# petim0/fly_bProject

Hardware: AMD Instinct MI355X
Metric: env-steps/sec (PPO rollout + update), 8192 envs per GPU (higher is better)
Workload: dtype f32 (optimizer step: fp16x2 operand split; rollout policy + critic: bf16x3 operand split; fp32 accumulate)

## Files before the change

### fly_bproject_amd/_lib.py

```python
import ctypes as C
import os

from .params import FlyParams

_HERE = os.path.dirname(os.path.abspath(__file__))
LIB_PATH = os.environ.get("FLYHIP_LIB") or os.path.join(_HERE, "libflyhip.so")
_lib = None


class FlyHipError(RuntimeError):
    pass


class FlyBuffers(C.Structure):
    _fields_ = [(n, C.c_void_p) for n in ("root", "dof_state", "targets", "contact", "pot", "prev_pot",
                                          "obs", "reward", "reset", "progress", "ep_return", "ep_length",
                                          "done_return", "done_length", "done_count")]


class FlyRenderConfig(C.Structure):
    _fields_ = [("width", C.c_int32), ("height", C.c_int32), ("fov_y_deg", C.c_float), ("cam_offset", C.c_float * 3),
                ("look_z", C.c_float)]


# ... 32 lines not shown
    "ppo_rollout_step": [_P, _P, _P, _P, _P, _P, _P, _I, _F, _F, _P, _P, _P, _P, _P, _P],
    "ppo_rollout_all": [_P, _P, _P, _P, _P, _P, _P, _F, _F, _P, _P, _P, _P, _I, _P, _P, _P, _P, _P],
    "ppo_rollout_bookkeeping": [_P, _L, _L, _P, _P, _F, _P, _I, _F, _F, _P, _P],
    "mlp_forward": [_P, _P, _P, _L, _P, _P, _P, _P, _P, _P, _P, _P],
    "mlp_forward_sample": [_P, _P, _P, _L, _P, _P, _I, _F, _F, _P, _P, _P, _P, _P, _P],
    "mlp_grad_workspace_floats": [],
    "mlp_backward_dx": [_P] * 10 + [_L, _F, _F, _P, _P, _P, _P, _P, _P, _P],
    "mlp_forward_backward": [_P] * 4 + [_L] + [_P] * 9 + [_F, _F] + [_P] * 6 + [_I, _P, _P, _P, _I, _P],
    "mlp_grad_w": [_P] * 8 + [_L, _P, _P, _P, _P, _P, _P, _I, _P],
    "mlp_fused_workspace_floats": [],
    "mlp_fused_grad": [_P] * 3 + [_P, _L] + [_P] * 5 + [_F, _F] + [_P] * 6 + [C.POINTER(_P), _P],
    "mlp_fused_h2_workspace_floats": [],
    "mlp_fused_grad_h2": [_P] * 5 + [_I, _P, _L] + [_P] * 5 + [_F, _F] + [_P] * 6 + [C.POINTER(_P), _P],
    "mlp_h2_rescale": [_P] * 7,
    "mlp_adam_step": [_P] * 10 + [_F, _F, _F, _F, _F, _F, _P, _I, _P, _P, _P, _P, _P, _P] + [_P] * 3 + [_I, _P],
    "dqn_eps_greedy": [_P, _P, _P, _F, _I, _P, _L, _P],
    "dqn_huber_td": [_P, _P, _P, _P, _P, _F, _I, _L, _P, _P, _P],
    "dqn_forward": [_P, _P, _P, _L, _P, _P],
    "dqn_act": [_P, _P, _P, _L, _P, _P, _F, _P, _P, _P],
    "dqn_td_step": [_P] * 10 + [_L, _F, _F] + [_P] * 7,
    "dqn_grad_workspace_floats": [],
    "dqn_grad_w": [_P] * 6 + [_L, _P, _P, _I, _P],
    "dqn_fused_workspace_floats": [],
    "dqn_fused_image_halves": [_L],
    "dqn_fused_update": [_P] * 6 + [_I, _L, _F, _F, _P, _P, _P, _P, _I, _P],
    "dqn_fused_h2_workspace_floats": [],
    "dqn_fused_h2_image_halves": [_L],
    "dqn_fused_update_h2": [_P] * 10 + [_I, _L, _F, _F, _P, _P, _P, _P, _I, _I, _P],
    "dqn_adam_soft_update": [_P] * 12 + [_F, _F, _F, _F, _F, _P, _P, _P, _P, _P, _P, _P],
    "dp_p2p_alloc": [_L, C.POINTER(_P)],
# ... 48 lines not shown
```

### fly_bproject_amd/csrc/flyhip_abi.hip

```cpp
#include <hip/hip_runtime.h>
#include <string.h>
#include <stdint.h>
#include <stdio.h>
#include <stdarg.h>
#include <new>
#include "flyhip.h"
#include "obs_norm.h"
#include "domain_rand.h"
#include <math.h>

extern "C" hipError_t flyhip_launch_env(int phases, const FlyConfig* dcfg, int n, const float* actions,
                                        const FlyBuffers* b, void* stream, int dr);
extern "C" hipError_t flyhip_launch_sample_logprob(const float* mu, const float* var, const float* eps,
                                                   float* act_out, float* logp_out, int64_t n, void* stream);
extern "C" hipError_t flyhip_launch_td_gae(const float* reward, const float* v, const float* v_next,
                                           const float* done, float gamma, float lambda, int64_t T, int64_t N,
                                           float* target_out, float* adv_out, int mode, void* stream);

extern "C" hipError_t flyhip_launch_mlp_forward(const float* P, const float* PF, const float* x, int64_t n, float* mu_out,
                                                float* v_out, float* out_save, float* h1_save, float* h2_save,
                                                float* h3_save, const uint16_t* PB, void* stream);

extern "C" hipError_t flyhip_launch_mlp_backward_dx(const float* PT, const float* out_saved, const float* h1,
                                                    const float* h2, const float* h3, const float* action,
// ... 27 lines not shown
                                                   int64_t n, const float* action, const float* old_logp, const float* adv,
                                                   const float* target, const float* var, float inv_batch, float clip,
                                                   float* workspace, float* grad_out, const float* norm_mask, float* norm_ws,
                                                   int* norm_step, float* loss_part, float* const* dump, void* stream);
extern "C" hipError_t flyhip_launch_mlp_grad_w(const float* x, const float* h1, const float* h2, const float* h3,
                                               const float* dz1, const float* dz2, const float* dz3, const float* dz4,
                                               int64_t n, float* workspace, float* grad_out, const float* norm_mask,
                                               float* norm_ws, int* norm_step, const int* err, int gemm_b3, void* stream);
extern "C" hipError_t flyhip_launch_mlp_adam(float* P, float* PF, float* PT, const int* idx_f, const int* idx_t,
                                             const float* G, const float* mask, float* m,
                                             float* v, int* step, float lr, float beta1, float beta2, float eps,
                                             float max_norm, float grad_scale, float* norm_ws, int norm_ready,
                                             uint16_t* PB, uint16_t* PTB, const int* idx_fb, const int* idx_tb,
                                             int* step_out, const int* grad_invalid, uint16_t* PH, uint16_t* PTH,
                                             float* h2_scales, int h2_period, void* stream);
extern "C" hipError_t flyhip_launch_mlp_h2_rescale(const float* P, const int* idx_fb, const int* idx_tb, uint16_t* PH, uint16_t* PTH,
                                                   float* h2_scales, void* stream);
extern "C" int64_t flyhip_mlp_fused_h2_workspace_floats(void);
extern "C" hipError_t flyhip_launch_mlp_fused_grad_h2(const float* P, const uint16_t* PH, const uint16_t* PTH, float* fsc, int* ovf,
                                                      int freeze, const float* x, int64_t n, const float* action,
                                                      const float* old_logp, const float* adv, const float* target, const float* var,
                                                      float inv_batch, float clip, float* workspace, float* grad_out,
                                                      const float* norm_mask, float* norm_ws, int* norm_step, float* loss_part,
                                                      float* const* dump, void* stream);

extern "C" hipError_t flyhip_launch_bookkeeping(const float* reward, int64_t n, float* score_acc, float score_scale,
                                                float* action_var, int nvar, float var_decay, float var_min,
                                                void* stream);

extern "C" hipError_t flyhip_launch_dqn_eps_greedy(const float* q, const float* coin_u, const float* rand_u, float epsilon,
// ... 527 lines not shown
{
    if (params_b3 && (!params_t_b3 || !idx_b3 || !idx_t_b3))
        return fail(FLY_E_ARG, "mlp_adam_step: params_b3 needs params_t_b3, idx_b3 and idx_t_b3");
    if (params_h2 && (!params_t_h2 || !h2_scales || !params_b3))
        return fail(FLY_E_ARG, "mlp_adam_step: params_h2 needs params_t_h2, h2_scales and the bf16x3 planes with their index maps");
    if (!params || !params_frag || !params_t_frag || !idx_frag || !idx_t_frag || !grad || !mask || !exp_avg ||
        !exp_avg_sq || !step || !norm_ws)
        return fail(FLY_E_ARG, "mlp_adam_step: null pointer");
    hipError_t e = flyhip_launch_mlp_adam(params, params_frag, params_t_frag, idx_frag, idx_t_frag, grad, mask, exp_avg, exp_avg_sq, step, lr, beta1, beta2,
                                          eps, max_norm, grad_scale, norm_ws, norm_ready, params_b3, params_t_b3, idx_b3, idx_t_b3,
                                          step_out, grad_invalid, params_h2, params_t_h2, h2_scales, h2_period, stream);
    if (e != hipSuccess) return hip_fail(e, "mlp_adam_step launch");
    return FLY_OK;
}

int dqn_eps_greedy(const float* q, const float* coin_u, const float* rand_u, float epsilon, int32_t A,
                   float* act_out, int64_t n, void* stream)
{
    if (!q || !coin_u || !rand_u || !act_out) return fail(FLY_E_ARG, "dqn_eps_greedy: null pointer");
    if (n <= 0 || A < 2) return fail(FLY_E_ARG, "dqn_eps_greedy: need n > 0 and A >= 2");
    hipError_t e = flyhip_launch_dqn_eps_greedy(q, coin_u, rand_u, epsilon, A, act_out, n, stream);
    if (e != hipSuccess) return hip_fail(e, "dqn_eps_greedy launch");
    return FLY_OK;
}

int dqn_huber_td(const float* q_table, const float* act, const float* reward, const float* q_next,
                 const float* done, float discount, int32_t A, int64_t B, float* dq, float* loss_part,
                 void* stream)
{
    if (!q_table || !act || !reward || !q_next || !done || !dq || !loss_part)
// ... 190 lines not shown
```

### fly_bproject_amd/csrc/mlp_adam.inc

```
constexpr int ADAM_THREADS = 1024;
constexpr int ADAM_WAVES = ADAM_THREADS / 64;
constexpr int ADAM_BLOCKS = (MLP_PACKED_FLOATS + ADAM_THREADS - 1) / ADAM_THREADS;

constexpr int H2_SINCE = 40;
constexpr int H2_WMAX = 64;
constexpr int H2_WMAX_SLOTS = (MLP_PACKED_FLOATS + 63) / 64;
constexpr int H2_TABLE_FLOATS = H2_WMAX + 2 * H2_WMAX_SLOTS;
__device__ __forceinline__ int h2_group_layer(int w)
{
    const int o = 64 * w;
    return o < MLP_OFF_B1 ? 0 : o < MLP_OFF_W2 ? -1 : o < MLP_OFF_B2 ? 1 : o < MLP_OFF_W3 ? -1 : o < MLP_OFF_B3 ? 2 : o < MLP_OFF_W4 ? -1
         : o < MLP_OFF_B4 ? 3 : -1;
}
__device__ __forceinline__ float h2_wave_max(float x)
{
    x = fmaxf(x, __builtin_bit_cast(float, __builtin_amdgcn_update_dpp(0, __builtin_bit_cast(int, x), 0xB1, 0xF, 0xF, true)));
    x = fmaxf(x, __builtin_bit_cast(float, __builtin_amdgcn_update_dpp(0, __builtin_bit_cast(int, x), 0x4E, 0xF, 0xF, true)));
    x = fmaxf(x, __builtin_bit_cast(float, __builtin_amdgcn_update_dpp(0, __builtin_bit_cast(int, x), 0x141, 0xF, 0xF, true)));
    x = fmaxf(x, __builtin_bit_cast(float, __builtin_amdgcn_update_dpp(0, __builtin_bit_cast(int, x), 0x140, 0xF, 0xF, true)));
    const int b = __builtin_bit_cast(int, x);
    return fmaxf(fmaxf(__builtin_bit_cast(float, __builtin_amdgcn_readlane(b, 0)), __builtin_bit_cast(float, __builtin_amdgcn_readlane(b, 16))),
                 fmaxf(__builtin_bit_cast(float, __builtin_amdgcn_readlane(b, 32)), __builtin_bit_cast(float, __builtin_amdgcn_readlane(b, 48))));
}
static_assert(MLP_OFF_B1 % 64 == 0 && MLP_OFF_W2 % 64 == 0 && MLP_OFF_B2 % 64 == 0 && MLP_OFF_W3 % 64 == 0 && MLP_OFF_B3 % 64 == 0 &&
// ... 153 lines not shown
            const _Float16 h1 = (_Float16)(ps - (float)h0);
            const u16 a = __builtin_bit_cast(u16, h0), b = __builtin_bit_cast(u16, h1);
            const int hf = (kf / 1536) * 1024 + kf % 1536;
            PH[hf] = a; PH[hf + 512] = b;
            if (kt >= 0) { const int ht = (kt / 1536) * 1024 + kt % 1536; PTH[ht] = a; PTH[ht + 512] = b; }
        }
    }
    if (PH) {
        const int w = i >> 6;
        float mw = 0.0f;
        if (h2_group_layer(w) >= 0) mw = h2_wave_max(fabsf(p));
        if ((tid & 63) == 0 && w < H2_WMAX_SLOTS) fsc[H2_WMAX + par * H2_WMAX_SLOTS + w] = mw;
    }
}

constexpr int H2_RESCALE_THREADS = 1024;
__global__ __launch_bounds__(H2_RESCALE_THREADS) void mlp_h2_rescale_kernel(const float* __restrict__ P, const int* __restrict__ idx_fb,
                                                                            const int* __restrict__ idx_tb, u16* __restrict__ PH,
                                                                            u16* __restrict__ PTH, float* __restrict__ fsc)
{
    __shared__ unsigned s_max[4];
    __shared__ float s_scale[4];
    const int tid = threadIdx.x;
    if (tid < 4) s_max[tid] = 0u;
    __syncthreads();
    float mine[4] = {0.0f, 0.0f, 0.0f, 0.0f};
    for (int i = tid; i < MLP_PACKED_FLOATS; i += H2_RESCALE_THREADS)
        if (idx_fb[i] >= 0) {
            const int layer = i < MLP_OFF_W2 ? 0 : i < MLP_OFF_W3 ? 1 : i < MLP_OFF_W4 ? 2 : 3;
            const float a = fabsf(P[i]);
// ... 42 lines not shown
```

### fly_bproject_amd/csrc/mlp_mfma.hip

```cpp
#include <hip/hip_runtime.h>
#include <stdint.h>
#include <type_traits>
#include <cstdio>
#include <cstdlib>
#include "flyhip.h"
#include "mlp_layout.h"
#include "obs_norm.h"
#include "domain_rand.h"

namespace {

#include "mlp_gemm.inc"
#include "fs_stamp.inc"
#include "mlp_forward.inc"
#include "mlp_backward.inc"
#include "mlp_grad_w.inc"
#include "mlp_fused_step.inc"
#include "mlp_adam.inc"
#include "fly_body.inc"

constexpr int RS_LDS_FLOATS = FWD_LDS_FLOATS > ENVS_PER_BLOCK * FLY_NUM_OBS ? FWD_LDS_FLOATS : ENVS_PER_BLOCK * FLY_NUM_OBS;
constexpr int RS_B3_LDS_FLOATS = FWD_B3_LDS_FLOATS > ENVS_PER_BLOCK * FLY_NUM_OBS ? FWD_B3_LDS_FLOATS : ENVS_PER_BLOCK * FLY_NUM_OBS;
static_assert(ENVS_PER_BLOCK == BM && BLOCK == THREADS, "one forward tile = one env block");
constexpr int NORM_LDS_FLOATS = OBS_NORM_TABLE + 1;
// ... 545 lines not shown
    } else if (norm_ready) {
        nparts = RED_BLOCKS;
        part_scale = grad_scale * grad_scale;
    } else {
        hipLaunchKernelGGL(mlp_adam_norm_kernel, dim3(ADAM_BLOCKS), dim3(ADAM_THREADS), 0, (hipStream_t)stream, G, mask,
                           grad_scale, norm_ws, step, grad_invalid);
        hipError_t e = hipGetLastError();
        if (e != hipSuccess) return e;
    }
    hipLaunchKernelGGL(mlp_adam_apply_kernel, dim3(ADAM_BLOCKS), dim3(ADAM_THREADS), 0, (hipStream_t)stream, P, PF, PT,
                       idx_f, idx_t, G, mask, m, v, step, lr, beta1, beta2, eps, max_norm, grad_scale, norm_ws, nparts,
                       part_scale, PB, PTB, idx_fb, idx_tb, step_out, grad_invalid, PH, PTH, h2_scales, h2_period);
    return hipGetLastError();
}

extern "C" hipError_t flyhip_launch_mlp_h2_rescale(const float* P, const int* idx_fb, const int* idx_tb, uint16_t* PH, uint16_t* PTH,
                                                   float* h2_scales, void* stream)
{
    hipLaunchKernelGGL(mlp_h2_rescale_kernel, dim3(1), dim3(H2_RESCALE_THREADS), 0, (hipStream_t)stream, P, idx_fb, idx_tb, PH, PTH, h2_scales);
    return hipGetLastError();
}
```

### fly_bproject_amd/policy.py

```python
import ctypes as C
import os

import torch

from . import _lib

IN, IN_PAD, H1, H2, H3, OUT, NACT = 73, 80, 256, 128, 128, 32, 18
OFF_W1 = 0
OFF_B1 = OFF_W1 + H1 * IN_PAD
OFF_W2 = OFF_B1 + H1
OFF_B2 = OFF_W2 + H2 * H1
OFF_W3 = OFF_B2 + H2
OFF_B3 = OFF_W3 + H3 * H2
OFF_W4 = OFF_B3 + H3
OFF_B4 = OFF_W4 + OUT * H3
PACKED = OFF_B4 + OUT
ERR_SLOT = OFF_W1 + 76
OFF_F1 = 0
OFF_F2 = OFF_F1 + H1 * IN_PAD
OFF_F3 = OFF_F2 + H2 * H1
OFF_F4 = OFF_F3 + H3 * H2
FRAG = OFF_F4 + OUT * H3
OFF_TF2 = 0
OFF_TF3 = OFF_TF2 + H1 * H2
# ... 109 lines not shown
        self._gemm = "bf16x3" if env_gemm in (None, "f16x2") else env_gemm
        self.gemm_infer = os.environ.get("FLY_GEMM_INFER", self._gemm)
        assert self._gemm in ("f32", "bf16x3") and self.gemm_infer in ("f32", "bf16x3")
        self.PB = torch.zeros(PB_HALVES, dtype=torch.int16, device=self.device)
        self.PTB = torch.zeros(PTB_HALVES, dtype=torch.int16, device=self.device)
        self._step_gemm = os.environ.get("FLY_STEP_GEMM", "f16x2" if env_gemm in (None, "f16x2") else "bf16x3")
        assert self._step_gemm in ("bf16x3", "f16x2")
        self.PH = torch.zeros(PH_HALVES, dtype=torch.int16, device=self.device)
        self.PTH = torch.zeros(PTH_HALVES, dtype=torch.int16, device=self.device)
        self.h2_scales = torch.zeros(H2_SCALE_FLOATS, dtype=torch.float32, device=self.device)
        self.h2_overflow = torch.zeros(1, dtype=torch.int32, device=self.device)
        self.h2_freeze = False
        self.h2_calibrated = False
        self.h2_suspended = False
        self.h2_overflows = 0
        self._h2_reset_scales()
        idx_fb, idx_tb = build_plane_maps()
        self.idx_fb = torch.from_numpy(idx_fb).to(self.device)
        self.idx_tb = torch.from_numpy(idx_tb).to(self.device)
        self._src_fb = torch.nonzero(self.idx_fb >= 0).squeeze(-1)
        self._dst_fb = self.idx_fb[self._src_fb].long()
        self._src_tb = torch.nonzero(self.idx_tb >= 0).squeeze(-1)
        self._dst_tb = self.idx_tb[self._src_tb].long()
        idx_f, idx_t = build_index_maps()
        self.idx_f = torch.from_numpy(idx_f).to(self.device)
        self.idx_t = torch.from_numpy(idx_t).to(self.device)
        self._src_f = torch.nonzero(self.idx_f >= 0).squeeze(-1)
        self._dst_f = self.idx_f[self._src_f].long()
        self._src_t = torch.nonzero(self.idx_t >= 0).squeeze(-1)
        self._dst_t = self.idx_t[self._src_t].long()
# ... 22 lines not shown
                params[k].data = view
        mask = torch.zeros(PACKED, dtype=torch.float32, device=self.device)
        for k, view in self.views.items():
            off = view.storage_offset()
            idx = torch.arange(PACKED, device=self.device).as_strided(view.shape, view.stride(), off)
            mask[idx.reshape(-1)] = 1.0
        self.grad_mask = mask
        assert int(mask.sum().item()) == 69587
        self.refresh()

    def refresh(self):
        with torch.no_grad():
            self.PF[self._dst_f] = self.P[self._src_f]
            self.PT[self._dst_t] = self.P[self._src_t]
            self._refresh_planes()
        self.h2_calibrated = False
        self.version += 1

    refresh_transposes = refresh

    def _refresh_planes(self):
        with torch.no_grad():
            for dst_buf, src, dst in ((self.PB, self._src_fb, self._dst_fb), (self.PTB, self._src_tb, self._dst_tb)):
                for term, plane in enumerate(split_bf16x3(self.P[src])):
                    dst_buf[dst + 512 * term] = plane

        if self.h2_live():
            self._refresh_planes_h2()

    def h2_live(self):
# ... 5 lines not shown
        s[4:8] = 2.0 ** 28
        s[H2_INV:H2_INV + 16] = 1.0 / s[:16]
        s[32:] = 0.0
        self.h2_scales.copy_(s)
        self.h2_calibrated = False

    def _refresh_planes_h2(self):
        if self.device.type != "cuda":
            return
        p = lambda t: C.c_void_p(t.data_ptr())
        _lib.check(self._lib.mlp_h2_rescale(p(self.P), p(self.idx_fb), p(self.idx_tb), p(self.PH), p(self.PTH), p(self.h2_scales),
                                            _lib.stream_ptr()), "mlp_h2_rescale")

    def _planes_live(self):
        return self._gemm == "bf16x3" or self.gemm_infer == "bf16x3"

    @property
    def step_gemm(self):
        return self._step_gemm if self._gemm == "bf16x3" else self._gemm

    @step_gemm.setter
    def step_gemm(self, mode):
        assert mode in ("bf16x3", "f16x2")
        was = self.h2_live()
        self._step_gemm = mode
        if self.h2_live() and not was:
            self._refresh_planes_h2()

    @property
    def gemm(self):
# ... 27 lines not shown
            return (None, None, None, C.c_int(0))
        p = lambda t: C.c_void_p(t.data_ptr())
        period = max(1, min(64, int(0.9 / (3.2 * self.lr))))
        return (p(self.PH), p(self.PTH), p(self.h2_scales), C.c_int(period))

    def pb_ptr(self):
        return C.c_void_p(self.PB.data_ptr()) if self.gemm == "bf16x3" else None

    def infer_pb_ptr(self):
        return C.c_void_p(self.PB.data_ptr()) if self.gemm_infer == "bf16x3" else None

    def ptb_ptr(self):
        return C.c_void_p(self.PTB.data_ptr()) if self.gemm == "bf16x3" else None

    def forward(self, x, want_mu=True, want_v=True, saves=None):
        lead = x.shape[:-1]
        x2 = x.reshape(-1, IN)
        if not x2.is_contiguous():
            x2 = x2.contiguous()
        n = x2.shape[0]
        mu = torch.empty((n, NACT), device=self.device) if want_mu else None
        v = torch.empty((n,), device=self.device) if want_v else None
        s = saves or {}
        ptr = lambda t: C.c_void_p(t.data_ptr()) if t is not None else None
        _lib.check(self._lib.mlp_forward(ptr(self.P), ptr(self.PF), ptr(x2), C.c_int64(n), ptr(mu), ptr(v), ptr(s.get("out")),
                                         ptr(s.get("h1")), ptr(s.get("h2")), ptr(s.get("h3")),
                                         self.pb_ptr() if saves else self.infer_pb_ptr(), _lib.stream_ptr()),
                   "mlp_forward")
        return (mu.view(*lead, NACT) if want_mu else None), (v.view(*lead, 1) if want_v else None)

# ... 39 lines not shown

    def update_can_be_refused(self):
        if self.fused_step and self.gemm == "bf16x3":
            return self.h2_live() and os.environ.get("FLY_H2_DIAG_NO_STEP_READ") != "1"
        return bool(self.fuse_fwd_bwd)

    def check_fused_launch(self):
        err = int(self.tile_wait_error.item())
        if err != 0:
            self.fuse_fwd_bwd = False
            self.fused_launch_failures = getattr(self, "fused_launch_failures", 0) + 1
            self.tile_wait_error.zero_()
        return err

    def minibatch_grad(self, x, action, old_logp, adv, target, var, clip, global_rows=None, fuse_norm=False, dump=False):
        n = x.shape[0]
        assert n <= self.max_rows and x.is_contiguous() and action.is_contiguous()
        for t in (old_logp, adv, target):
            assert t.is_contiguous() and t.numel() == n
        s, d = self.saves, self.dz
        p = lambda t: C.c_void_p(t.data_ptr())
        st = _lib.stream_ptr()
        inv_b = 1.0 / float(global_rows if global_rows else n)
        if self.fused_step and self.gemm == "bf16x3":
            return self._fused_grad(x, action, old_logp, adv, target, var, clip, inv_b, fuse_norm, dump)
        if dump:
            raise ValueError("dump=True is a debugging aid of the fused step")
        if self.fuse_fwd_bwd:
            if self._epoch >= (1 << 27) - 1:
                self._tile_flags.zero_()
# ... 64 lines not shown
                    "tracked) + mlp_adam_step, gemm=bf16x3, step_gemm=f16x2")
        if self.fused_step and self.gemm == "bf16x3":
            return "mlp_fused_grad (ONE persistent launch: forward + loss + dX chain + dW per tile, slabs reduced) + mlp_adam_step, gemm=bf16x3"
        if self.fuse_fwd_bwd:
            return "mlp_forward_backward (one launch, per-tile flags) + mlp_grad_w (+reduce) + mlp_adam_step, gemm=" + self.gemm
        return "mlp_forward + mlp_backward_dx + mlp_grad_w (+reduce) + mlp_adam_step, gemm=" + self.gemm

    def loss_value(self, n):
        parts = self.loss_part[: (n + 31) // 32].sum(0)
        return (parts[0] + parts[1]) / n

    @property
    def step(self):
        return self._step2[self._step_idx:self._step_idx + 1]

    def adam_step(self, grad_scale=1.0, norm_ready=False, self_norm=False, grad_invalid=None):
        p = lambda t: C.c_void_p(t.data_ptr())
        self.version += 1
        self.steps_issued += 1
        step_in = self.step
        step_out = None
        if self_norm:
            self._step_idx ^= 1
            step_out = p(self.step)
        _lib.check(self._lib.mlp_adam_step(p(self.P), p(self.PF), p(self.PT), p(self.idx_f), p(self.idx_t), p(self.G),
                                           p(self.grad_mask), p(self.exp_avg),
                                           p(self.exp_avg_sq), p(step_in), C.c_float(self.lr),
                                           C.c_float(self.betas[0]), C.c_float(self.betas[1]), C.c_float(self.eps),
                                           C.c_float(self.max_norm), C.c_float(grad_scale), p(self._norm_ws),
                                           C.c_int(1 if norm_ready else 0), *self._plane_args(), step_out,
                                           p(grad_invalid) if grad_invalid is not None else None, *self._h2_args(), _lib.stream_ptr()),
                   "mlp_adam_step")
```

### fly_bproject_amd/ppo.py

```python
import ctypes as C
import collections
import os

import torch
import torch.nn as nn
import torch.nn.functional as F

from . import _lib
from .fly import Fly
from .params import NUM_DOF


class Net(nn.Module):

    def __init__(self, num_obs, num_act):
        super().__init__()
        self.shared_net = nn.Sequential(nn.Linear(num_obs, 256), nn.ELU(), nn.Linear(256, 128), nn.ELU())
        self.to_mean = nn.Sequential(nn.Linear(128, 64), nn.ELU(), nn.Linear(64, num_act), nn.ELU())
        self.to_value = nn.Sequential(nn.Linear(128, 64), nn.ELU(), nn.Linear(64, 1))

    _policy = None

    def pi(self, x):
        if self._policy is not None and not torch.is_grad_enabled():
# ... 87 lines not shown
            raise ValueError("obs_clip must be > 0 (got %r)" % self.obs_clip)
        self.use_graph = bool(getattr(args, "graph", False))
        want = getattr(args, "persistent_rollout", None)
        if want is None:
            want = os.environ.get("FLY_PERSISTENT_ROLLOUT", "1") != "0"
        self.persistent_rollout = bool(want) and T <= 4096 and not bool(getattr(args, "graph", False))
        self._reset_rows = self._progress_rows = None
        self._graphs = {}
        self._graphs_form = getattr(self.env, "launch_form", 0)
        self._fwd_args = None
        self._score_acc = torch.zeros((), device=dev)
        want_async = getattr(args, "async_log", None)
        if want_async is None:
            want_async = os.environ.get("FLY_ASYNC_LOG", "1") != "0"
        self._async_log = bool(want_async) and dev.type == "cuda"
        self._log_q = collections.deque()
        self.log_throughput = bool(getattr(args, "log_throughput", False))
        self._rate_mark = None
        self._pending_step = None
        self.env.bind_obs(self._obs_ring[0])

        self.score = 0
        self.run_step = 0
        self.optim_step = 0

        self.net = Net(self.env.num_obs, self.env.num_act).to(dev)
        loaded_rms = {}
        if getattr(self.args, "load", False):
            print("loaded from: ", str(self.args.load_path))
            sd = torch.load(self.args.load_path, map_location=dev, weights_only=True)
# ... 212 lines not shown
        sync_grads = self.world_size > 1 and self.dp_mode == "grad_allreduce"
        slices = [(j - mc, j) for _ in range(self.epoch) for j in range(mc, self.rollout_size, mc)]
        self.prepare()

        def run(todo):
            for k, j in todo:
                pol.minibatch_grad(obs[k:j].view(rows, self.num_obs), action[k:j].view(rows, self.num_acts),
                                   old_log_prob[k:j].view(rows), advantage[k:j].view(rows),
                                   target[k:j].view(rows), self._action_var, self.clip,
                                   fuse_norm=not sync_grads)
                if sync_grads:
                    if self._p2p is not None:
                        self._p2p.allreduce_(pol.G)
                    else:
                        dist.all_reduce(pol.G, op=dist.ReduceOp.SUM)
                pol.adam_step(grad_scale=1.0 / self.world_size if sync_grads else 1.0, norm_ready=not sync_grads,
                              self_norm=sync_grads, grad_invalid=self._p2p.err if (sync_grads and self._p2p is not None) else None)

        self._check_step_counter()
        if pol.h2_live() and pol.fused_step and not pol.h2_calibrated:
            k, j = slices[0]
            pol.calibrate_h2(obs[k:j].view(rows, self.num_obs), action[k:j].view(rows, self.num_acts), old_log_prob[k:j].view(rows),
                             advantage[k:j].view(rows), target[k:j].view(rows), self._action_var, self.clip)
        run(slices)
        if self._p2p is not None and not self._p2p.check():
            raise _lib.FlyHipError("dp_allreduce_p2p: a rank never published its gradient (bounded wait expired; "
                                   "FLY_P2P_POLL_LOG2 raises the budget, --dp_allreduce rccl avoids the kernel)")
        if not pol.update_can_be_refused():
            if self._p2p is None and self._async_log:
                host = torch.empty(1, dtype=pol.step.dtype, pin_memory=True)
                host.copy_(pol.step, non_blocking=True)
                ev = torch.cuda.Event()
# ... 114 lines not shown
            step.append((P(pol.P.data_ptr()), P(pol.PF.data_ptr()), P(self._obs_rows[t].data_ptr()),
                         P(self._eps_all[t].data_ptr()), var_ptr, C.c_int(t), C.c_float(self._var_decay), self._var_min,
                         P(self._act_rows[t].data_ptr()), P(self.all_log_prob[t].data_ptr()), P(self._v_ring[t].data_ptr()),
                         pol.infer_pb_ptr(), base_ptr))
            bufs.append((self._obs_rows[t + 1].data_ptr(), self._reward_rows[t].data_ptr()))
        self._fwd_args, self._buf_ptrs, self._step_args = fwd, bufs, step
        self._graphs = {}
        self.fuse_rollout_step = os.environ.get("FLY_FUSE_ROLLOUT_STEP", "1") != "0"
        self._args_infer_gemm = pol.gemm_infer
        if self.normalize_obs and not self.fuse_rollout_step and not self.persistent_rollout:
            raise _lib.FlyHipError("normalize_obs: the two-launch rollout step (FLY_FUSE_ROLLOUT_STEP=0, mlp_forward_sample) does not "
                                   "normalise observations; use the one-launch step")

    def _launch_step(self, t):
        lib, env = self._lib, self.env
        st = C.c_void_p(torch.cuda.current_stream().cuda_stream)
        if t == 0:
            self._eps_all.normal_(generator=self._gen)
            self._rows_applied.zero_()
        env.obs_buf, env.reward_buf = self._obs_rows[t + 1], self._reward_rows[t]
        env._bufs.obs, env._bufs.reward = self._buf_ptrs[t]
        if self.fuse_rollout_step:
            rc = lib.ppo_rollout_step(env._handle, C.byref(env._bufs), *self._step_args[t], st)
        else:
            rc = lib.mlp_forward_sample(*self._fwd_args[t], st)
            rc |= lib.fly_step(env._handle, C.c_void_p(self._act_rows[t].data_ptr()), C.byref(env._bufs), st)
        if rc:
            _lib.check(rc, "rollout step")
        self._after_step(t)
        if env.recorder is not None:
            env.recorder.capture(t)
        env.render_count += 1

    def _launch_rollout(self):
        P = C.c_void_p
        pol, env, T = self.policy, self.env, self.rollout_size
        self._eps_all.normal_(generator=self._gen)
        self._rows_applied.zero_()
        if self._reset_rows is None:
            n = int(self.args.num_envs)
            self._reset_rows = torch.zeros((T, n), dtype=torch.long, device=self.device)
            self._progress_rows = torch.zeros((T, n), dtype=torch.long, device=self.device)
        rec = env.recorder
        if rec is not None:
            rec.buffer(T)
            rec.flush()
            _lib.check(self._lib.fly_set_pose_record(env._handle, P(rec.poses.data_ptr())), "fly_set_pose_record")
        _lib.check(self._lib.ppo_rollout_all(
            env._handle, C.byref(env._bufs), P(pol.P.data_ptr()), P(pol.PF.data_ptr()), P(self._obs_ring.data_ptr()),
            P(self._eps_all.data_ptr()), P(self._action_var.data_ptr()), C.c_float(self._var_decay), self._var_min,
            P(self.all_acts.data_ptr()), P(self.all_log_prob.data_ptr()), P(self._v_ring.data_ptr()),
# ... 100 lines not shown
                self._launch_step(t)
            else:
                if t == 0:
                    key = bool(self.args.testing)
                    g = self._graphs.get(key)
                    if g is None:
                        g = torch.cuda.CUDAGraph()
                        g.register_generator_state(self._gen)
                        torch.cuda.synchronize(self.device)
                        count = self.env.render_count
                        with torch.cuda.graph(g):
                            for tt in range(self.rollout_size):
                                self._launch_step(tt)
                        self.env.render_count = count
                        self._graphs[key] = g
                    g.replay()
                self.env.obs_buf, self.env.reward_buf = self._obs_rows[t + 1], self._reward_rows[t]
                self.env._bufs.obs, self.env._bufs.reward = self._buf_ptrs[t]
                self._after_step(t)
                self.env.render_count += 1
            if rec is not None:
                rec.reached(t, step_s)
                if t + 1 == self.rollout_size:
                    rec.flush()

        if t + 1 == self.rollout_size:
            self._flush_bookkeeping()
            if not self.args.testing:
                self._emit("Training")
                self.update()
# ... 44 lines not shown
```

### include/flyhip.h

```cpp
#ifndef FLYHIP_H
#define FLYHIP_H

#include <stdint.h>

#ifdef __cplusplus
extern "C" {
#endif

#define FLY_NUM_DOF 18
#define FLY_NUM_OBS 73
#define FLY_NUM_LEGS 6
#define FLY_NUM_ABDOMEN 5
#define FLY_NUM_CONTACT 11
#define FLY_ROOT_DIM 13
#define FLY_POSE_FLOATS 25
#define FLY_OBS_NORM_TABLE 147
#define FLY_OBS_NORM_SET 147
#define FLY_OBS_NORM_SETS 256
#define FLY_DR_PARAMS 6
#define FLY_DR_ROW 8

#define FLY_OK 0
#define FLY_E_ARG (-1)
#define FLY_E_HIP (-2)
// ... 187 lines not shown
                   float inv_batch, float clip, float* workspace, float* grad, const float* norm_mask, float* norm_ws,
                   int32_t* norm_step, float* loss_part, float* const* debug_dump, void* stream);
int mlp_adam_step(float* params, float* params_frag, float* params_t_frag, const int32_t* idx_frag,
                  const int32_t* idx_t_frag, const float* grad, const float* mask, float* exp_avg,
                  float* exp_avg_sq, int32_t* step, float lr, float beta1, float beta2, float eps,
                  float max_norm, float grad_scale, float* norm_ws, int32_t norm_ready,
                  uint16_t* params_b3, uint16_t* params_t_b3, const int32_t* idx_b3,
                  const int32_t* idx_t_b3, int32_t* step_out, const int32_t* grad_invalid,
                  uint16_t* params_h2, uint16_t* params_t_h2, float* h2_scales, int32_t h2_period, void* stream);

#define MLP_PH_HALVES_ABI 147456
#define MLP_PTH_HALVES_ABI 106496
#define MLP_H2_SCALE_FLOATS_ABI 2386
int mlp_h2_rescale(const float* params, const int32_t* idx_b3, const int32_t* idx_t_b3, uint16_t* params_h2, uint16_t* params_t_h2,
                   float* h2_scales, void* stream);
int64_t mlp_fused_h2_workspace_floats(void);
int mlp_fused_grad_h2(const float* params, const uint16_t* params_h2, const uint16_t* params_t_h2, float* h2_scales,
                      int32_t* h2_overflow, int32_t freeze, const float* x, int64_t n, const float* action,
                      const float* old_logp, const float* adv, const float* target, const float* var, float inv_batch,
                      float clip, float* workspace, float* grad, const float* norm_mask, float* norm_ws, int32_t* norm_step,
                      float* loss_part, float* const* debug_dump, void* stream);


int dqn_eps_greedy(const float* q, const float* coin_u, const float* rand_u, float epsilon, int32_t A,
                   float* act_out, int64_t n, void* stream);
int dqn_huber_td(const float* q_table, const float* act, const float* reward, const float* q_next,
                 const float* done, float discount, int32_t A, int64_t B, float* dq, float* loss_part,
                 void* stream);

#define DQN_QB_HALVES_ABI 282624
// ... 51 lines not shown
```

Baseline: 67.99 million.

## Add lean Adam step that defers derived weight copy refresh to end of update

Adds a lean Adam kernel for the single-rank fp16x2 update loop. Per minibatch it writes only the master params, the Adam moments and the h2 fp16 split planes, using block-local transposes. The fp32 fragment, transpose and bf16x3 plane copies are marked stale and rebuilt once by a new refresh kernel after the update epochs finish. This cuts per-step scatter and write traffic in the optimizer. In exchange it adds staleness tracking and guards, plus a fallback refresh when a non-h2 gradient path needs the derived copies.

```diff
diff --git a/fly_bproject_amd/_lib.py b/fly_bproject_amd/_lib.py
--- a/fly_bproject_amd/_lib.py
+++ b/fly_bproject_amd/_lib.py
@@ -70,6 +70,8 @@
     "mlp_fused_grad_h2": [_P] * 5 + [_I, _P, _L] + [_P] * 5 + [_F, _F] + [_P] * 6 + [C.POINTER(_P), _P],
     "mlp_h2_rescale": [_P] * 7,
     "mlp_adam_step": [_P] * 10 + [_F, _F, _F, _F, _F, _F, _P, _I, _P, _P, _P, _P, _P, _P] + [_P] * 3 + [_I, _P],
+    "mlp_adam_step_lean": [_P] * 6 + [_F, _F, _F, _F, _F, _F, _P, _I, _P, _P, _P, _P, _I, _P],
+    "mlp_refresh_derived": [_P] * 10,
     "dqn_eps_greedy": [_P, _P, _P, _F, _I, _P, _L, _P],
     "dqn_huber_td": [_P, _P, _P, _P, _P, _F, _I, _L, _P, _P, _P],
     "dqn_forward": [_P, _P, _P, _L, _P, _P],
diff --git a/fly_bproject_amd/csrc/flyhip_abi.hip b/fly_bproject_amd/csrc/flyhip_abi.hip
--- a/fly_bproject_amd/csrc/flyhip_abi.hip
+++ b/fly_bproject_amd/csrc/flyhip_abi.hip
@@ -65,6 +65,12 @@
                                              uint16_t* PB, uint16_t* PTB, const int* idx_fb, const int* idx_tb,
                                              int* step_out, const int* grad_invalid, uint16_t* PH, uint16_t* PTH,
                                              float* h2_scales, int h2_period, void* stream);
+extern "C" hipError_t flyhip_launch_mlp_adam_lean(float* P, const float* G, const float* mask, float* m, float* v, int* step, float lr,
+                                                  float beta1, float beta2, float eps, float max_norm, float grad_scale,
+                                                  float* norm_ws, int norm_ready, const int* grad_invalid, uint16_t* PH,
+                                                  uint16_t* PTH, float* h2_scales, int h2_period, void* stream);
+extern "C" hipError_t flyhip_launch_mlp_refresh_derived(const float* P, float* PF, float* PT, const int* idx_f, const int* idx_t,
+                                                        uint16_t* PB, uint16_t* PTB, const int* idx_fb, const int* idx_tb, void* stream);
 extern "C" hipError_t flyhip_launch_mlp_h2_rescale(const float* P, const int* idx_fb, const int* idx_tb, uint16_t* PH, uint16_t* PTH,
                                                    float* h2_scales, void* stream);
 extern "C" int64_t flyhip_mlp_fused_h2_workspace_floats(void);
@@ -622,6 +628,33 @@
     return FLY_OK;
 }
 
+int mlp_adam_step_lean(float* params, const float* grad, const float* mask, float* exp_avg, float* exp_avg_sq, int32_t* step,
+                       float lr, float beta1, float beta2, float eps, float max_norm, float grad_scale, float* norm_ws,
+                       int32_t norm_ready, const int32_t* grad_invalid, uint16_t* params_h2, uint16_t* params_t_h2, float* h2_scales,
+                       int32_t h2_period, void* stream)
+{
+    if (!params || !grad || !mask || !exp_avg || !exp_avg_sq || !step || !norm_ws || !params_h2 || !params_t_h2 || !h2_scales)
+        return fail(FLY_E_ARG, "mlp_adam_step_lean: null pointer");
+    if (h2_period < 1) return fail(FLY_E_ARG, "mlp_adam_step_lean: h2_period must be >= 1");
+    hipError_t e = flyhip_launch_mlp_adam_lean(params, grad, mask, exp_avg, exp_avg_sq, step, lr, beta1, beta2, eps, max_norm, grad_scale,
+                                               norm_ws, norm_ready, grad_invalid, params_h2, params_t_h2, h2_scales, h2_period, stream);
+    if (e != hipSuccess) return hip_fail(e, "mlp_adam_step_lean launch");
+    return FLY_OK;
+}
+
+int mlp_refresh_derived(const float* params, float* params_frag, float* params_t_frag, const int32_t* idx_frag,
+                        const int32_t* idx_t_frag, uint16_t* params_b3, uint16_t* params_t_b3, const int32_t* idx_b3,
+                        const int32_t* idx_t_b3, void* stream)
+{
+    if (!params || !params_frag || !params_t_frag || !idx_frag || !idx_t_frag) return fail(FLY_E_ARG, "mlp_refresh_derived: null pointer");
+    if (params_b3 && (!params_t_b3 || !idx_b3 || !idx_t_b3))
+        return fail(FLY_E_ARG, "mlp_refresh_derived: params_b3 needs params_t_b3, idx_b3 and idx_t_b3");
+    hipError_t e = flyhip_launch_mlp_refresh_derived(params, params_frag, params_t_frag, idx_frag, idx_t_frag, params_b3, params_t_b3,
+                                                     idx_b3, idx_t_b3, stream);
+    if (e != hipSuccess) return hip_fail(e, "mlp_refresh_derived launch");
+    return FLY_OK;
+}
+
 int dqn_eps_greedy(const float* q, const float* coin_u, const float* rand_u, float epsilon, int32_t A,
                    float* act_out, int64_t n, void* stream)
 {
diff --git a/fly_bproject_amd/csrc/mlp_adam.inc b/fly_bproject_amd/csrc/mlp_adam.inc
--- a/fly_bproject_amd/csrc/mlp_adam.inc
+++ b/fly_bproject_amd/csrc/mlp_adam.inc
@@ -191,6 +191,257 @@
     }
 }
 
+constexpr int LEAN_ELEMS = 8;
+constexpr int LEAN_THREADS = 128;
+constexpr int LEAN_BLOCK_ELEMS = LEAN_THREADS * LEAN_ELEMS;
+constexpr int LEAN_B_W1 = MLP_H1 * MLP_IN_PAD / LEAN_BLOCK_ELEMS, LEAN_B_W2 = MLP_H2 * MLP_H1 / LEAN_BLOCK_ELEMS,
+              LEAN_B_W3 = MLP_H3 * MLP_H2 / LEAN_BLOCK_ELEMS, LEAN_B_W4 = MLP_OUT * MLP_H3 / LEAN_BLOCK_ELEMS;
+constexpr int LEAN_BLOCKS = LEAN_B_W1 + LEAN_B_W2 + LEAN_B_W3 + LEAN_B_W4 + 4;
+static_assert(MLP_H1 * MLP_IN_PAD % LEAN_BLOCK_ELEMS == 0 && MLP_H2 * MLP_H1 % LEAN_BLOCK_ELEMS == 0 &&
+              MLP_H3 * MLP_H2 % LEAN_BLOCK_ELEMS == 0 && MLP_OUT * MLP_H3 % LEAN_BLOCK_ELEMS == 0 && MLP_H1 <= LEAN_BLOCK_ELEMS,
+              "weight regions are whole blocks, a bias region fits one");
+static_assert(LEAN_BLOCK_ELEMS % MLP_H1 == 0 && LEAN_BLOCK_ELEMS / MLP_H1 == 4 && LEAN_BLOCK_ELEMS / MLP_H2 == 8 && MLP_H2 == MLP_H3,
+              "a block is 4 rows of W2, 8 rows of W3 / W4");
+static_assert(MLP_PACKED_FLOATS % LEAN_ELEMS == 0 && LEAN_THREADS % 64 == 0 && ADAM_THREADS % LEAN_THREADS == 0, "lean apply: whole groups, whole waves");
+static_assert(RED_BLOCKS <= ADAM_THREADS && ADAM_BLOCKS <= ADAM_THREADS, "one norm partial per lane of mlp_adam_apply_kernel");
+static_assert(MLP_IN_PAD % 16 == 0 && MLP_H1 % 16 == 0 && MLP_H2 % 16 == 0 && MLP_H3 % 16 == 0 && MLP_OFF_PB2 % 1536 == 0 &&
+              MLP_OFF_PB3 % 1536 == 0 && MLP_OFF_PB4 % 1536 == 0 && MLP_OFF_PTB3 % 1536 == 0 && MLP_OFF_PTB4 % 1536 == 0,
+              "plane regions are whole [term][lane][8] blocks");
+
+__device__ __forceinline__ int h2_fwd_word(int layer, int n, int k)
+{
+    int blk;
+    if (layer == 0) blk = MLP_OFF_PB1 / 1536 + (n >> 5) * (MLP_IN_PAD / 16) + (k >> 4);
+    else if (layer == 1) blk = MLP_OFF_PB2 / 1536 + (k >> 7) * (MLP_H2 * 128 / 512) + (n >> 5) * (128 / 16) + ((k & 127) >> 4);
+    else if (layer == 2) blk = MLP_OFF_PB3 / 1536 + (n >> 5) * (MLP_H2 / 16) + (k >> 4);
+    else blk = MLP_OFF_PB4 / 1536 + (n >> 5) * (MLP_H3 / 16) + (k >> 4);
+    return blk * 1024 + ((((k & 15) >> 3) * 32 + (n & 31)) << 3) + (k & 7);
+}
+__device__ __forceinline__ int h2_bwd_word(int layer, int n, int k, int N)
+{
+    const int base = layer == 1 ? MLP_OFF_PTB2 / 1536 : layer == 2 ? MLP_OFF_PTB3 / 1536 : MLP_OFF_PTB4 / 1536;
+    return (base + (k >> 5) * (N >> 4) + (n >> 4)) * 1024 + ((((n & 15) >> 3) * 32 + (k & 31)) << 3) + (n & 7);
+}
+
+__global__ __launch_bounds__(LEAN_THREADS) void mlp_adam_apply_lean_kernel(float* __restrict__ P, const float* __restrict__ G,
+                                                                           const float* __restrict__ mask, float* __restrict__ m,
+                                                                           float* __restrict__ v, const int* __restrict__ step,
+                                                                           float lr, float beta1, float beta2, float eps,
+                                                                           float max_norm, float grad_scale,
+                                                                           float* __restrict__ norm_ws, int nparts, float part_scale,
+                                                                           const int* __restrict__ grad_invalid,
+                                                                           u16* __restrict__ PH, u16* __restrict__ PTH,
+                                                                           float* __restrict__ fsc, int h2_period)
+{
+    __shared__ float s_coef, s_step_size, s_bc2_sqrt;
+    __shared__ float red[ADAM_WAVES];
+    __shared__ float s_wscale[4];
+    __shared__ unsigned s_wmax[4];
+    const int tid = threadIdx.x;
+    const float err_mark = G[MLP_ERR_SLOT];
+    const int err_word = grad_invalid ? *grad_invalid : 0;
+    int b = blockIdx.x, e0, e1;
+    if (b < LEAN_B_W1) { e0 = MLP_OFF_W1 + b * LEAN_BLOCK_ELEMS; e1 = MLP_OFF_B1; }
+    else if ((b -= LEAN_B_W1) == 0) { e0 = MLP_OFF_B1; e1 = MLP_OFF_W2; }
+    else if ((b -= 1) < LEAN_B_W2) { e0 = MLP_OFF_W2 + b * LEAN_BLOCK_ELEMS; e1 = MLP_OFF_B2; }
+    else if ((b -= LEAN_B_W2) == 0) { e0 = MLP_OFF_B2; e1 = MLP_OFF_W3; }
+    else if ((b -= 1) < LEAN_B_W3) { e0 = MLP_OFF_W3 + b * LEAN_BLOCK_ELEMS; e1 = MLP_OFF_B3; }
+    else if ((b -= LEAN_B_W3) == 0) { e0 = MLP_OFF_B3; e1 = MLP_OFF_W4; }
+    else if ((b -= 1) < LEAN_B_W4) { e0 = MLP_OFF_W4 + b * LEAN_BLOCK_ELEMS; e1 = MLP_OFF_B4; }
+    else { e0 = MLP_OFF_B4; e1 = MLP_PACKED_FLOATS; }
+    const int i0 = e0 + tid * LEAN_ELEMS;
+    const bool live = i0 < e1;
+    const int grp = i0 / LEAN_ELEMS;
+    __shared__ uint4 s_t[2][LEAN_THREADS];
+    const float4 z4 = make_float4(0.0f, 0.0f, 0.0f, 0.0f);
+    float4 mk4[2] = {z4, z4}, g4[2] = {z4, z4}, m4[2] = {z4, z4}, v4[2] = {z4, z4}, p4[2] = {z4, z4};
+    if (live) {
+#pragma unroll
+        for (int h = 0; h < 2; ++h) {
+            mk4[h] = reinterpret_cast<const float4*>(mask + i0)[h];
+            g4[h] = reinterpret_cast<const float4*>(G + i0)[h];
+            m4[h] = reinterpret_cast<const float4*>(m + i0)[h];
+            v4[h] = reinterpret_cast<const float4*>(v + i0)[h];
+            p4[h] = reinterpret_cast<const float4*>(P + i0)[h];
+        }
+    }
+    constexpr int LEAN_WAVES = LEAN_THREADS / 64, CHUNKS = ADAM_WAVES / LEAN_WAVES;
+    float part[CHUNKS];
+#pragma unroll
+    for (int j = 0; j < CHUNKS; ++j) {
+        const int b = ((tid >> 6) + j * LEAN_WAVES) * 64 + (tid & 63);
+        part[j] = b < nparts ? norm_ws[1 + b] : 0.0f;
+    }
+    const int step_now = *step;
+    const float s0 = fsc[H2_SINCE], s1 = fsc[H2_SINCE + 1];
+    const float4 ws4 = *reinterpret_cast<const float4*>(fsc + 8);
+    if (err_mark != 0.0f || err_word != 0) return;
+#pragma unroll
+    for (int o = 32; o > 0; o >>= 1)
+#pragma unroll
+        for (int j = 0; j < CHUNKS; ++j) part[j] += __shfl_down(part[j], o, 64);
+    if ((tid & 63) == 0)
+#pragma unroll
+        for (int j = 0; j < CHUNKS; ++j) red[(tid >> 6) + j * LEAN_WAVES] = part[j];
+    const int par = step_now & 1;
+    const int since = (int)(par ? s0 : s1);
+    const bool rescale = since >= h2_period;
+    if (blockIdx.x == 0 && tid == 0) fsc[H2_SINCE + par] = rescale ? 1.0f : (float)(since + 1);
+    if (!rescale && tid == 0) { s_wscale[0] = ws4.x; s_wscale[1] = ws4.y; s_wscale[2] = ws4.z; s_wscale[3] = ws4.w; }
+    if (rescale) {
+        if (tid < 4) s_wmax[tid] = 0u;
+        __syncthreads();
+        float mx[4] = {0.0f, 0.0f, 0.0f, 0.0f};
+        const float* wm = fsc + H2_WMAX + (par ^ 1) * H2_WMAX_SLOTS;
+        for (int w = tid; w < H2_WMAX_SLOTS; w += LEAN_THREADS) {
+            const int l = h2_group_layer(w);
+            const float a = wm[w];
+#pragma unroll
+            for (int k = 0; k < 4; ++k) mx[k] = l == k ? fmaxf(mx[k], a) : mx[k];
+        }
+#pragma unroll
+        for (int k = 0; k < 4; ++k) {
+            float mm = mx[k];
+#pragma unroll
+            for (int o = 32; o > 0; o >>= 1) mm = fmaxf(mm, __shfl_xor(mm, o, 64));
+            if ((tid & 63) == 0 && mm > 0.0f) atomicMax(&s_wmax[k], __float_as_uint(mm));
+        }
+        __syncthreads();
+        if (tid < 4) {
+            const float mm = fminf(fmaxf(__uint_as_float(s_wmax[tid]), 0x1p-4f), 0x1p60f);
+            const float sc = ldexpf(1.0f, 11 - ilogbf(mm));
+            s_wscale[tid] = sc;
+            if (blockIdx.x == 0) { fsc[8 + tid] = sc; fsc[16 + 8 + tid] = 1.0f / sc; }
+        }
+    }
+    __syncthreads();
+    if (tid == 0) {
+        float t = 0.0f;
+        for (int w = 0; w < ADAM_WAVES; ++w) t += red[w];
+        t *= part_scale;
+        const float norm = sqrtf(t);
+        const float coef = max_norm / (norm + 1e-6f);
+        s_coef = coef < 1.0f ? coef : 1.0f;
+        if (blockIdx.x == 0) norm_ws[0] = norm;
+        const float ts = (float)step_now;
+        const float bc1 = 1.0f - powf(beta1, ts);
+        const float bc2 = 1.0f - powf(beta2, ts);
+        s_step_size = lr / bc1;
+        s_bc2_sqrt = sqrtf(bc2);
+    }
+    __syncthreads();
+    float amax = 0.0f;
+    int t_layer = 0;
+    if (live) {
+        const float coef = s_coef * grad_scale;
+        const float step_size = s_step_size;
+        const float bc2_sqrt = s_bc2_sqrt;
+        const float mk_[8] = {mk4[0].x, mk4[0].y, mk4[0].z, mk4[0].w, mk4[1].x, mk4[1].y, mk4[1].z, mk4[1].w};
+        const float g_[8] = {g4[0].x, g4[0].y, g4[0].z, g4[0].w, g4[1].x, g4[1].y, g4[1].z, g4[1].w};
+        const float m_[8] = {m4[0].x, m4[0].y, m4[0].z, m4[0].w, m4[1].x, m4[1].y, m4[1].z, m4[1].w};
+        const float v_[8] = {v4[0].x, v4[0].y, v4[0].z, v4[0].w, v4[1].x, v4[1].y, v4[1].z, v4[1].w};
+        const float p_[8] = {p4[0].x, p4[0].y, p4[0].z, p4[0].w, p4[1].x, p4[1].y, p4[1].z, p4[1].w};
+        float mo[8], vo[8], po[8];
+#pragma unroll
+        for (int e = 0; e < 8; ++e) {
+            const float g = g_[e] * coef * mk_[e];
+            const float mi = beta1 * m_[e] + (1.0f - beta1) * g;
+            const float vi = beta2 * v_[e] + (1.0f - beta2) * g * g;
+            const float denom = sqrtf(vi) / bc2_sqrt + eps;
+            mo[e] = mi; vo[e] = vi;
+            po[e] = p_[e] - mk_[e] * (step_size * (mi / denom));
+        }
+#pragma unroll
+        for (int h = 0; h < 2; ++h) {
+            reinterpret_cast<float4*>(m + i0)[h] = make_float4(mo[4 * h], mo[4 * h + 1], mo[4 * h + 2], mo[4 * h + 3]);
+            reinterpret_cast<float4*>(v + i0)[h] = make_float4(vo[4 * h], vo[4 * h + 1], vo[4 * h + 2], vo[4 * h + 3]);
+            reinterpret_cast<float4*>(P + i0)[h] = make_float4(po[4 * h], po[4 * h + 1], po[4 * h + 2], po[4 * h + 3]);
+        }
+        int layer = -1, off = 0, K = 1;
+        if (i0 < MLP_OFF_B1) { layer = 0; off = MLP_OFF_W1; K = MLP_IN_PAD; }
+        else if (i0 >= MLP_OFF_W2 && i0 < MLP_OFF_B2) { layer = 1; off = MLP_OFF_W2; K = MLP_H1; }
+        else if (i0 >= MLP_OFF_W3 && i0 < MLP_OFF_B3) { layer = 2; off = MLP_OFF_W3; K = MLP_H2; }
+        else if (i0 >= MLP_OFF_W4 && i0 < MLP_OFF_B4) { layer = 3; off = MLP_OFF_W4; K = MLP_H3; }
+        if (layer >= 0) {
+            const int n = (i0 - off) / K, k0 = (i0 - off) - n * K;
+            const float sc = s_wscale[layer];
+            u16 a[8], b[8];
+#pragma unroll
+            for (int e = 0; e < 8; ++e) {
+                amax = fmaxf(amax, fabsf(po[e]));
+                const float ps = po[e] * sc;
+                const _Float16 h0 = (_Float16)ps;
+                const _Float16 h1 = (_Float16)(ps - (float)h0);
+                a[e] = __builtin_bit_cast(u16, h0); b[e] = __builtin_bit_cast(u16, h1);
+            }
+            const int hf = h2_fwd_word(layer, n, k0);
+            const uint4 qa = make_uint4(a[0] | (unsigned)a[1] << 16, a[2] | (unsigned)a[3] << 16, a[4] | (unsigned)a[5] << 16,
+                                        a[6] | (unsigned)a[7] << 16);
+            const uint4 qb = make_uint4(b[0] | (unsigned)b[1] << 16, b[2] | (unsigned)b[3] << 16, b[4] | (unsigned)b[5] << 16,
+                                        b[6] | (unsigned)b[7] << 16);
+            *reinterpret_cast<uint4*>(PH + hf) = qa;
+            *reinterpret_cast<uint4*>(PH + hf + 512) = qb;
+            if (layer >= 1) { s_t[0][tid] = qa; s_t[1][tid] = qb; t_layer = layer; }
+        }
+    }
+    t_layer = __shfl(t_layer, 0, 64);
+    if (t_layer > 0) {
+        __syncthreads();
+        const u16* sh = reinterpret_cast<const u16*>(s_t);
+        const int off = t_layer == 1 ? MLP_OFF_W2 : t_layer == 2 ? MLP_OFF_W3 : MLP_OFF_W4;
+        const int N = t_layer == 1 ? MLP_H2 : t_layer == 2 ? MLP_H3 : MLP_OUT;
+        if (t_layer == 1) {
+            const int n0 = (e0 - off) / MLP_H1;
+#pragma unroll
+            for (int q = 0; q < 2; ++q) {
+                const int k = tid + q * LEAN_THREADS;
+#pragma unroll
+                for (int term = 0; term < 2; ++term) {
+                    const u16* row = sh + term * (LEAN_THREADS * 8) + k;
+                    const uint2 w = make_uint2(row[0] | (unsigned)row[MLP_H1] << 16, row[2 * MLP_H1] | (unsigned)row[3 * MLP_H1] << 16);
+                    *reinterpret_cast<uint2*>(PTH + h2_bwd_word(1, n0, k, N) + 512 * term) = w;
+                }
+            }
+        } else {
+            const int n0 = (e0 - off) / MLP_H2, k = tid;
+#pragma unroll
+            for (int term = 0; term < 2; ++term) {
+                const u16* row = sh + term * (LEAN_THREADS * 8) + k;
+                const uint4 w = make_uint4(row[0] | (unsigned)row[128] << 16, row[256] | (unsigned)row[384] << 16,
+                                           row[512] | (unsigned)row[640] << 16, row[768] | (unsigned)row[896] << 16);
+                *reinterpret_cast<uint4*>(PTH + h2_bwd_word(t_layer, n0, k, N) + 512 * term) = w;
+            }
+        }
+    }
+    amax = fmaxf(amax, __shfl_xor(amax, 1, 64));
+    amax = fmaxf(amax, __shfl_xor(amax, 2, 64));
+    amax = fmaxf(amax, __shfl_xor(amax, 4, 64));
+    if (live && (tid & 7) == 0 && (grp >> 3) < H2_WMAX_SLOTS) fsc[H2_WMAX + par * H2_WMAX_SLOTS + (grp >> 3)] = amax;
+}
+
+constexpr int REFRESH_THREADS = 256;
+constexpr int REFRESH_BLOCKS = 146;
+__global__ __launch_bounds__(REFRESH_THREADS) void mlp_refresh_derived_kernel(const float* __restrict__ P, float* __restrict__ PF,
+                                                                              float* __restrict__ PT, const int* __restrict__ idx_f,
+                                                                              const int* __restrict__ idx_t, u16* __restrict__ PB,
+                                                                              u16* __restrict__ PTB, const int* __restrict__ idx_fb,
+                                                                              const int* __restrict__ idx_tb)
+{
+    for (int i = blockIdx.x * REFRESH_THREADS + threadIdx.x; i < MLP_PACKED_FLOATS; i += REFRESH_BLOCKS * REFRESH_THREADS) {
+        const float p = P[i];
+        const int jf = idx_f[i], jt = idx_t[i];
+        if (jf >= 0) PF[jf] = p;
+        if (jt >= 0) PT[jt] = p;
+        if (PB) {
+            u16 a, b, c;
+            split3(p, a, b, c);
+            const int kf = idx_fb[i], kt = idx_tb[i];
+            if (kf >= 0) { PB[kf] = a; PB[kf + 512] = b; PB[kf + 1024] = c; }
+            if (kt >= 0) { PTB[kt] = a; PTB[kt + 512] = b; PTB[kt + 1024] = c; }
+        }
+    }
+}
+
 constexpr int H2_RESCALE_THREADS = 1024;
 __global__ __launch_bounds__(H2_RESCALE_THREADS) void mlp_h2_rescale_kernel(const float* __restrict__ P, const int* __restrict__ idx_fb,
                                                                             const int* __restrict__ idx_tb, u16* __restrict__ PH,
diff --git a/fly_bproject_amd/csrc/mlp_mfma.hip b/fly_bproject_amd/csrc/mlp_mfma.hip
--- a/fly_bproject_amd/csrc/mlp_mfma.hip
+++ b/fly_bproject_amd/csrc/mlp_mfma.hip
@@ -583,6 +583,36 @@
     return hipGetLastError();
 }
 
+extern "C" hipError_t flyhip_launch_mlp_adam_lean(float* P, const float* G, const float* mask, float* m, float* v, int* step, float lr,
+                                                  float beta1, float beta2, float eps, float max_norm, float grad_scale,
+                                                  float* norm_ws, int norm_ready, const int* grad_invalid, uint16_t* PH,
+                                                  uint16_t* PTH, float* h2_scales, int h2_period, void* stream)
+{
+    int nparts = ADAM_BLOCKS;
+    float part_scale = 1.0f;
+    if (norm_ready) {
+        nparts = RED_BLOCKS;
+        part_scale = grad_scale * grad_scale;
+    } else {
+        hipLaunchKernelGGL(mlp_adam_norm_kernel, dim3(ADAM_BLOCKS), dim3(ADAM_THREADS), 0, (hipStream_t)stream, G, mask,
+                           grad_scale, norm_ws, step, grad_invalid);
+        hipError_t e = hipGetLastError();
+        if (e != hipSuccess) return e;
+    }
+    hipLaunchKernelGGL(mlp_adam_apply_lean_kernel, dim3(LEAN_BLOCKS), dim3(LEAN_THREADS), 0, (hipStream_t)stream, P, G, mask, m, v,
+                       step, lr, beta1, beta2, eps, max_norm, grad_scale, norm_ws, nparts, part_scale, grad_invalid, PH, PTH,
+                       h2_scales, h2_period);
+    return hipGetLastError();
+}
+
+extern "C" hipError_t flyhip_launch_mlp_refresh_derived(const float* P, float* PF, float* PT, const int* idx_f, const int* idx_t,
+                                                        uint16_t* PB, uint16_t* PTB, const int* idx_fb, const int* idx_tb, void* stream)
+{
+    hipLaunchKernelGGL(mlp_refresh_derived_kernel, dim3(REFRESH_BLOCKS), dim3(REFRESH_THREADS), 0, (hipStream_t)stream, P, PF, PT,
+                       idx_f, idx_t, PB, PTB, idx_fb, idx_tb);
+    return hipGetLastError();
+}
+
 extern "C" hipError_t flyhip_launch_mlp_h2_rescale(const float* P, const int* idx_fb, const int* idx_tb, uint16_t* PH, uint16_t* PTH,
                                                    float* h2_scales, void* stream)
 {
diff --git a/fly_bproject_amd/policy.py b/fly_bproject_amd/policy.py
--- a/fly_bproject_amd/policy.py
+++ b/fly_bproject_amd/policy.py
@@ -147,6 +147,7 @@
         self.h2_calibrated = False
         self.h2_suspended = False
         self.h2_overflows = 0
+        self.derived_stale = False
         self._h2_reset_scales()
         idx_fb, idx_tb = build_plane_maps()
         self.idx_fb = torch.from_numpy(idx_fb).to(self.device)
@@ -199,6 +200,7 @@
             self.PF[self._dst_f] = self.P[self._src_f]
             self.PT[self._dst_t] = self.P[self._src_t]
             self._refresh_planes()
+        self.derived_stale = False
         self.h2_calibrated = False
         self.version += 1
 
@@ -234,6 +236,17 @@
 
     def _planes_live(self):
         return self._gemm == "bf16x3" or self.gemm_infer == "bf16x3"
+
+    def need_derived(self, what):
+        if self.derived_stale:
+            raise _lib.FlyHipError("%s reads the derived weight copies (PF / PT / PB / PTB), which are stale: lean optimizer steps "
+                                   "were issued and refresh_derived() has not run" % what)
+
+    def refresh_derived(self):
+        p = lambda t: C.c_void_p(t.data_ptr())
+        _lib.check(self._lib.mlp_refresh_derived(p(self.P), p(self.PF), p(self.PT), p(self.idx_f), p(self.idx_t), *self._plane_args(),
+                                                 _lib.stream_ptr()), "mlp_refresh_derived")
+        self.derived_stale = False
 
     @property
     def step_gemm(self):
@@ -291,6 +304,7 @@
         return C.c_void_p(self.PTB.data_ptr()) if self.gemm == "bf16x3" else None
 
     def forward(self, x, want_mu=True, want_v=True, saves=None):
+        self.need_derived("mlp_forward")
         lead = x.shape[:-1]
         x2 = x.reshape(-1, IN)
         if not x2.is_contiguous():
@@ -360,6 +374,8 @@
         return err
 
     def minibatch_grad(self, x, action, old_logp, adv, target, var, clip, global_rows=None, fuse_norm=False, dump=False):
+        if self.derived_stale and not (self.fused_step and self.h2_live() and not self.h2_suspended):
+            self.refresh_derived()
         n = x.shape[0]
         assert n <= self.max_rows and x.is_contiguous() and action.is_contiguous()
         for t in (old_logp, adv, target):
@@ -454,10 +470,21 @@
     def step(self):
         return self._step2[self._step_idx:self._step_idx + 1]
 
-    def adam_step(self, grad_scale=1.0, norm_ready=False, self_norm=False, grad_invalid=None):
-        p = lambda t: C.c_void_p(t.data_ptr())
+    def adam_step(self, grad_scale=1.0, norm_ready=False, self_norm=False, grad_invalid=None, lean=False):
+        p = lambda t: C.c_void_p(t.data_ptr())
+        if lean and (self_norm or not self.h2_live()):
+            raise _lib.FlyHipError("adam_step(lean=True) is the fp16x2 update loop's single-rank step (no self_norm form)")
         self.version += 1
         self.steps_issued += 1
+        if lean:
+            self.derived_stale = True
+            _lib.check(self._lib.mlp_adam_step_lean(p(self.P), p(self.G), p(self.grad_mask), p(self.exp_avg), p(self.exp_avg_sq),
+                                                    p(self.step), C.c_float(self.lr), C.c_float(self.betas[0]),
+                                                    C.c_float(self.betas[1]), C.c_float(self.eps), C.c_float(self.max_norm),
+                                                    C.c_float(grad_scale), p(self._norm_ws), C.c_int(1 if norm_ready else 0),
+                                                    p(grad_invalid) if grad_invalid is not None else None, *self._h2_args(),
+                                                    _lib.stream_ptr()), "mlp_adam_step_lean")
+            return
         step_in = self.step
         step_out = None
         if self_norm:
diff --git a/fly_bproject_amd/ppo.py b/fly_bproject_amd/ppo.py
--- a/fly_bproject_amd/ppo.py
+++ b/fly_bproject_amd/ppo.py
@@ -125,6 +125,7 @@
         if want_async is None:
             want_async = os.environ.get("FLY_ASYNC_LOG", "1") != "0"
         self._async_log = bool(want_async) and dev.type == "cuda"
+        self.adam_lean = os.environ.get("FLY_ADAM_LEAN", "1") != "0"
         self._log_q = collections.deque()
         self.log_throughput = bool(getattr(args, "log_throughput", False))
         self._rate_mark = None
@@ -367,8 +368,12 @@
                         self._p2p.allreduce_(pol.G)
                     else:
                         dist.all_reduce(pol.G, op=dist.ReduceOp.SUM)
+                lean = self.adam_lean and pol.h2_live() and pol.fused_step and not pol.h2_suspended and not sync_grads
                 pol.adam_step(grad_scale=1.0 / self.world_size if sync_grads else 1.0, norm_ready=not sync_grads,
-                              self_norm=sync_grads, grad_invalid=self._p2p.err if (sync_grads and self._p2p is not None) else None)
+                              self_norm=sync_grads, grad_invalid=self._p2p.err if (sync_grads and self._p2p is not None) else None,
+                              lean=lean)
+            if pol.derived_stale:
+                pol.refresh_derived()
 
         self._check_step_counter()
         if pol.h2_live() and pol.fused_step and not pol.h2_calibrated:
@@ -513,6 +518,7 @@
 
     def _launch_step(self, t):
         lib, env = self._lib, self.env
+        self.policy.need_derived("the rollout step")
         st = C.c_void_p(torch.cuda.current_stream().cuda_stream)
         if t == 0:
             self._eps_all.normal_(generator=self._gen)
@@ -534,6 +540,7 @@
     def _launch_rollout(self):
         P = C.c_void_p
         pol, env, T = self.policy, self.env, self.rollout_size
+        pol.need_derived("the rollout launch")
         self._eps_all.normal_(generator=self._gen)
         self._rows_applied.zero_()
         if self._reset_rows is None:
@@ -664,6 +671,7 @@
                                 self._launch_step(tt)
                         self.env.render_count = count
                         self._graphs[key] = g
+                    self.policy.need_derived("the rollout graph")
                     g.replay()
                 self.env.obs_buf, self.env.reward_buf = self._obs_rows[t + 1], self._reward_rows[t]
                 self.env._bufs.obs, self.env._bufs.reward = self._buf_ptrs[t]
diff --git a/include/flyhip.h b/include/flyhip.h
--- a/include/flyhip.h
+++ b/include/flyhip.h
@@ -225,6 +225,13 @@
 #define MLP_H2_SCALE_FLOATS_ABI 2386
 int mlp_h2_rescale(const float* params, const int32_t* idx_b3, const int32_t* idx_t_b3, uint16_t* params_h2, uint16_t* params_t_h2,
                    float* h2_scales, void* stream);
+int mlp_adam_step_lean(float* params, const float* grad, const float* mask, float* exp_avg, float* exp_avg_sq, int32_t* step,
+                       float lr, float beta1, float beta2, float eps, float max_norm, float grad_scale, float* norm_ws,
+                       int32_t norm_ready, const int32_t* grad_invalid, uint16_t* params_h2, uint16_t* params_t_h2, float* h2_scales,
+                       int32_t h2_period, void* stream);
+int mlp_refresh_derived(const float* params, float* params_frag, float* params_t_frag, const int32_t* idx_frag,
+                        const int32_t* idx_t_frag, uint16_t* params_b3, uint16_t* params_t_b3, const int32_t* idx_b3,
+                        const int32_t* idx_t_b3, void* stream);
 int64_t mlp_fused_h2_workspace_floats(void);
 int mlp_fused_grad_h2(const float* params, const uint16_t* params_h2, const uint16_t* params_t_h2, float* h2_scales,
                       int32_t* h2_overflow, int32_t freeze, const float* x, int64_t n, const float* action,
```

New measurement: 68.47 million (median of 6 runs). About the same (+0.7%).
